# huyhoang17/DB_text_minimal

Measured on AMD Instinct MI355X. Metric: train images/sec @640x640 bs=16/GPU, higher is better.
Workload: dtype f32

## Files before the change

### db_text_minimal_amd/_lib.py

```python
import ctypes
import os
import subprocess

_HERE = os.path.dirname(os.path.abspath(__file__))
LIB_PATH = os.environ.get('DBN_LIB_PATH') or os.path.join(_HERE, 'libdbnet_hip.so')
CSRC = os.path.join(_HERE, 'csrc')

_P, _I, _L, _F, _D = ctypes.c_void_p, ctypes.c_int, ctypes.c_long, ctypes.c_float, ctypes.c_double

SIGNATURES = {
    'dbn_pack_weights': 'piiiiiipp',
    'dbn_igemm_panel_floats': 'iiiiii',
    'dbn_igemm_packed_floats': 'ii',
    'dbn_igemm_f32': 'pppp' + 'i' * 14 + 'p',
    'dbn_igemm_tile_config': 'ii',
    'dbn_igemm_tile_config_ns': 'iii',
    'dbn_conv_bn_ws_floats': 'iiiiii',
    'dbn_pack_weights_batched': 'piip',
    'dbn_igemm_splitk_plan': 'iiii',
    'dbn_igemm_splitk_plan_ns': 'iiiii',
    'dbn_igemm_splitk_f32': 'pppp' + 'i' * 16 + 'pp',
    'dbn_deform_im2col': 'ppp' + 'i' * 11 + 'p',
    'dbn_deform_col2im': 'ppppp' + 'i' + 'p' + 'i' * 11 + 'p',
    'dbn_deform_col2im_ws_bytes': 'i' * 8,
# ... 85 lines not shown
    'dbn_head_tail_bwd': 'p' * 21 + 'iiii' + 'ff' + 'pp',
    'dbn_db_loss_ws_bytes': '',
    'dbn_db_loss_fwd': 'pp' + 'iiii' + 'ffdf' + 'pppp',
    'dbn_db_loss_sum_fwd': 'pp' + 'iiii' + 'ffdf' + 'pppp',
    'dbn_db_loss_frac_fwd': 'pp' + 'iiii' + 'ffdf' + 'i' + 'pppp',
    'dbn_db_loss_bwd': 'pppp' + 'ff' + 'iiii' + 'pp',
    'dbn_db_loss_ohem_ws_bytes': 'iii',
    'dbn_db_loss_ohem_fwd': 'pp' + 'iiii' + 'ffdf' + 'pppp',
    'dbn_db_loss_ohem_bwd': 'ppppp' + 'ff' + 'iiii' + 'pp',
    'dbn_pixel_confusion': 'plppiiifpp',
    'dbn_adam_step': 'pppp' + 'l' + 'ffff' + 'i' + 'f' + 'p',
    'dbn_clock_probe': 'pip',
    'dbn_has_experiments': '',
    'dbn_wall_clock_khz': '',
}
SIGNATURES.update({
    'dbn_igemm_t': 'ii' + 'pppp' + 'i' * 14 + 'i' + 'p' + 'p',
    'dbn_conv_bn_t': 'i' + SIGNATURES['dbn_conv_bn_f32'],
    'dbn_pyramid_conv_t': 'i' + SIGNATURES['dbn_pyramid_conv_f32'],
    'dbn_pyramid_conv_from_t': 'ii' + SIGNATURES['dbn_pyramid_conv_f32'],
    'dbn_igemm_bn_rows': 'i' * 15,
    'dbn_igemm_bnsums_t': 'ii' + 'pppp' + 'i' * 14 + 'ppppppp' + 'pppp' + 'p' + 'p',
    'dbn_igemm_bn_final_counters': 'ii',
    'dbn_igemm_bn_final_group_floats': 'ii',
    'dbn_wgrad_t': 'ii' + 'pppp' + 'i' * 12 + 'f' + 'p',
    'dbn_wgrad_phase_t': 'iii' + 'pppp' + 'i' * 12 + 'f' + 'p',
    'dbn_wgrad_reduce_describe': 'ii' + 'pppp' + 'i' * 12 + 'f' + 'p',
    'dbn_wgrad_reduce_many': 'ppiiip',
    'dbn_wgrad_tile_config': 'ii',
    'dbn_set_wgrad_variant': 'i',
    'dbn_set_convt_kernel': 'i',
    'dbn_igemm_splitk_slab_floats': 'iiiii',
    'dbn_wgrad_kernel_config': 'iiiii',
    'dbn_wgrad_kernel_config_hw': 'i' * 12,
    'dbn_set_patch_conv': 'i',
    'dbn_set_wres16': 'i',
    'dbn_set_pyramid_wide': 'i',
    'dbn_pyramid_wide_would_run': 'iiiiii',
    'dbn_conv_bn_set_final': 'pp',
    'dbn_conv_bn_final_group_doubles': 'ii',
    'dbn_wres16_would_run': 'iiiiiiiii',
    'dbn_mfma_sustained': 'ippip',
    'dbn_mfma_sustained_flops': 'ii',
    'dbn_set_stagger': 'i',
    'dbn_winograd_eligible': 'iiiii',
    'dbn_winograd_panel_floats': 'ii',
    'dbn_winograd_pack': 'piiiipp',
    'dbn_winograd_rows': 'iii',
    'dbn_winograd_pack_batched': 'pip',
    'dbn_winograd_dgrad_bnsums_f32': 'ppp' + 'iiiiii' + 'pppp' + 'ppp' + 'pppp' + 'p' + 'p',
    'dbn_winograd_ws_floats': 'iiii',
    'dbn_winograd_wgrad_eligible': 'iiiiii',
    'dbn_winograd_wgrad_linear': 'ii',
    'dbn_winograd_wgrad_slab_floats': 'iiiii',
    'dbn_winograd_wgrad_f32': 'ipppppp' + 'iiiiii' + 'fp',
    'dbn_winograd_conv_bn_act_f32': 'pppppp' + 'iiiii' + 'pp' + 'ff' + 'ppppppp' + 'p',
    'dbn_winograd_conv_bn_f32': 'pppp' + 'iiiii' + 'pp' + 'ff' + 'ppppppp' + 'p',
    'dbn_set_phase_priority': 'i',
    'dbn_set_winograd_persistent': 'i',
    'dbn_set_winograd_stagger': 'i',
    'dbn_set_winograd_blocks_per_barrier': 'i',
    'dbn_fold_bn_eval': 'pilppppp' + 'f' + 'ppp',
    'dbn_igemm_act_t': 'ii' + 'pppp' + 'i' + 'p' + 'i' * 13 + 'p',
    'dbn_winograd_conv_act_f32': 'pppp' + 'i' + 'p' + 'iiiii' + 'p',
    'dbn_pyramid_conv_act_t': 'ii' + 'p' * 9 + 'i' + 'p' + 'i' * 6 + 'p',
    'dbn_set_trace': 'pl',
    'dbn_igemm_kernel_config': 'i' * 16,
    'dbn_split3': 'pplp',
    'dbn_deform_im2col_t': 'i' + SIGNATURES['dbn_deform_im2col'],
    'dbn_deform_col2im_t': 'i' + SIGNATURES['dbn_deform_col2im'],
    'dbn_deform_col2im_gather_t': 'i' + SIGNATURES['dbn_deform_col2im'],
    'dbn_deform_col2im_gather_ws_bytes': 'iii',
    'dbn_deform_offset_absmax_t': 'iplpp',
    'dbn_pw16_eligible': 'iiiiii',
    'dbn_pw16_panel_bytes': '',
    'dbn_pw16_pack': 'ipipp',
    'dbn_pw16_act_t': 'ipppipiiiip',
    'dbn_set_head_tail_wide': 'i',
    'dbn_stem16_pool_eligible': 'iiii',
    'dbn_stem16_conv_bn_relu_pool_t': 'ipppppiiip',
    'dbn_head16_eligible': 'iiii',
    'dbn_head16_tail_eval_t': 'i' + 'p' * 15 + 'iii' + 'p',
    'dbn_cast_f32': 'ipplp',
    'dbn_pack_weights_t': 'ip' + 'i' * 7 + 'pp',
    'dbn_igemm_panel_floats_t': 'i' * 8,
    'dbn_bn_train_stats_t': 'i' + SIGNATURES['dbn_bn_train_stats'],
    'dbn_bn_apply_t': 'i' + SIGNATURES['dbn_bn_apply'],
    'dbn_bn_backward_t': 'ipi' + SIGNATURES['dbn_bn_backward_ex'][1:],
    'dbn_col_sum_t': 'i' + SIGNATURES['dbn_col_sum'],
    'dbn_bnrelu_maxpool_fwd_t': 'i' + SIGNATURES['dbn_bnrelu_maxpool_fwd'],
    'dbn_bnrelu_maxpool_bwd_t': 'i' + SIGNATURES['dbn_bnrelu_maxpool_bwd'][:-1] + 'pppp',
    'dbn_maxpool_bwd_parts': 'iiii',
    'dbn_bnrelu_maxpool_fwd_arg_t': 'ipppppp' + 'iiii' + 'p',
    'dbn_maxpool_bn_backward_ws_floats': 'iiii',
    'dbn_maxpool_bn_backward_t': 'i' + 'p' * 10 + 'iiii' + 'f' + 'pp',
    'dbn_nearest_up_fwd_t': 'i' + SIGNATURES['dbn_nearest_up_fwd'],
    'dbn_nearest_up_bwd_t': 'i' + SIGNATURES['dbn_nearest_up_bwd'],
    'dbn_nchw3_to_nhwc4_t': 'i' + SIGNATURES['dbn_nchw3_to_nhwc4'],
    'dbn_nchw3_to_nhwc4_packed_t': 'i' + SIGNATURES['dbn_nchw3_to_nhwc4'],
    'dbn_nchw3_to_nhwc16_and_4_t': 'ipppiiip',
    'dbn_convt16_rows': '',
    'dbn_convt16_panel_bytes': '',
    'dbn_convt16_eligible': 'iiiiii',
    'dbn_convt16_pack': 'ippp',
    'dbn_convt16_bn_t': 'ippppiii' + 'pp' + 'ff' + 'ppppppp' + 'p',
    'dbn_stem16_padded_h': 'i',
# ... 86 lines not shown
```

### db_text_minimal_amd/csrc/winograd_wgrad_f32.hip

```cpp
#include "igemm_common.h"
#include <algorithm>
#ifndef DBN_WWG_PIPE
#define DBN_WWG_PIPE 1
#endif
#ifndef DBN_WWG_EXP
#define DBN_WWG_EXP 0
#endif

namespace {

constexpr int WG_XPX = 180, WG_XROW = 18, WG_YPX = 128, WG_YROW = 16;

struct WinoWgradParams {
    const float* x;
    const float* dy;
    float* slab;
    int N, H, W, Cx, Cy;
    int nob, nib;
    int tw, gpi, groups;
    int nsplit;
    unsigned x_bytes, dy_bytes;
    const float *x_scale, *x_shift;
};

constexpr int WL_XPX = 336, WL_YPX = 240;
template <bool LIN>
__global__ __launch_bounds__(512) __attribute__((amdgpu_waves_per_eu(2, 2))) void winograd_wgrad_f32_kernel(const WinoWgradParams p) {
    constexpr int XPX = LIN ? WL_XPX : WG_XPX, YPX = LIN ? WL_YPX : WG_YPX;
    constexpr int XCH = XPX * 16, YCH = YPX * 16;
    constexpr int NXP = (XCH + 511) / 512, NYP = (YCH + 511) / 512;
    constexpr int NBUF = LIN ? 1 : 2;
    __shared__ f32x4 smem[NBUF * (XCH + YCH)];
    const int tid = threadIdx.x, lane = tid & 63, wave = __builtin_amdgcn_readfirstlane(tid >> 6);
    const int li = lane & 31, lh = lane >> 5;
    const int irow = wave & 3, oh = wave >> 2;
    const int nsub = p.nob * p.nib;
    const int b = dbn_xcd_remap(blockIdx.x, gridDim.x);
    const int split = b / nsub, sub = b - split * nsub;
    const int ob = sub / p.nib, ib = sub - ob * p.nib;
    const int g0 = (int)((long)split * p.groups / p.nsplit), g1 = (int)((long)(split + 1) * p.groups / p.nsplit);
    const __amdgpu_buffer_rsrc_t rsX = __builtin_amdgcn_make_buffer_rsrc(const_cast<float*>(p.x), 0, p.x_bytes, 0x00020000);
    const __amdgpu_buffer_rsrc_t rsY = __builtin_amdgcn_make_buffer_rsrc(const_cast<float*>(p.dy), 0, p.dy_bytes, 0x00020000);
    const int TW = (p.W + 1) >> 1, TI = ((p.H + 1) >> 1) * TW;
    const int prow = LIN ? 2 * TW + 2 : WG_XROW, yrow = LIN ? 2 * TW : WG_YROW;
    const float rTW = 1.0f / (float)TW;

    unsigned xrel[NXP], yrel[NYP];
    int xpos[NXP], ypos[NYP];
#pragma unroll
    for (int j = 0; j < NXP; ++j) {
        const int idx = tid + j * 512, pix = idx >> 4, ch = idx & 15;
        int py, px;
        if constexpr (LIN) divmod24(pix, prow, 1.0f / (float)prow, py, px);
        else { py = pix / WG_XROW; px = pix - py * WG_XROW; }
        xrel[j] = (unsigned)((py * p.W + px) * p.Cx + ch * 4) * 4u;
        xpos[j] = idx < XCH ? (py | (px << 8)) : -1;
    }
#pragma unroll
    for (int j = 0; j < NYP; ++j) {
        const int idx = tid + j * 512, pix = idx >> 4, ch = idx & 15;
        int py, px;
        if constexpr (LIN) divmod24(pix, yrow, 1.0f / (float)yrow, py, px);
        else { py = pix >> 4; px = pix & 15; }
        yrel[j] = (unsigned)((py * p.W + px) * p.Cy + ch * 4) * 4u;
        ypos[j] = idx < YCH ? (py | (px << 8)) : -1;
    }
    f32x4 rx[NXP], ry[LIN ? 1 : NYP];
    const bool act = p.x_scale != nullptr;
    f32x4 asc_ = {0.f, 0.f, 0.f, 0.f}, ash_ = {0.f, 0.f, 0.f, 0.f};
    if (act && !LIN) {
        asc_ = *reinterpret_cast<const f32x4*>(p.x_scale + ib * 64 + (tid & 15) * 4);
        ash_ = *reinterpret_cast<const f32x4*>(p.x_shift + ib * 64 + (tid & 15) * 4);
    }
    unsigned xstatic = 0;
#pragma unroll
    for (int j = 0; j < NXP; ++j) xstatic |= (unsigned)(xpos[j] >= 0) << j;
    unsigned xvalid = 0;
    int t0 = 0, tr0 = 0;
    auto geometry = [&](int g, int& n, int& hs0, int& ws0, int& xrows) {
        n = g / p.gpi;
        const int t = g - n * p.gpi;
        if constexpr (LIN) {
            const int tfirst = t * 32, tlast = min(tfirst + 31, TI - 1);
            const int r0_ = tfirst / TW, r1_ = tlast / TW;
            hs0 = 2 * r0_ - 1;
            ws0 = -1;
            xrows = 2 * (r1_ - r0_ + 1) + 2;
        } else {
            const int ty = t / p.tw, tx = t - ty * p.tw;
            hs0 = ty * 8 - 1;
            ws0 = tx * 16 - 1;
            xrows = 10;
        }
    };
    auto load_x = [&](int g) {
        int n, hs0, ws0, xrows;
        geometry(g, n, hs0, ws0, xrows);
        const unsigned bx = (unsigned)(((n * p.H + hs0) * p.W + ws0) * p.Cx + ib * 64) * 4u;
        if (!LIN && hs0 >= 0 && hs0 + 10 <= p.H && ws0 >= 0 && ws0 + WG_XROW <= p.W) {
#pragma unroll
            for (int j = 0; j < NXP; ++j) rx[j] = buffer_load_f32x4(rsX, xpos[j] >= 0 ? bx + xrel[j] : OOB_OFFSET);
            xvalid = xstatic;
            return;
        }
#pragma unroll
        for (int j = 0; j < NXP; ++j) {
            const int py = xpos[j] & 255, px = xpos[j] >> 8;
            const bool v = xpos[j] >= 0 && py < xrows && (unsigned)(hs0 + py) < (unsigned)p.H && (unsigned)(ws0 + px) < (unsigned)p.W;
            rx[j] = buffer_load_f32x4(rsX, v ? bx + xrel[j] : OOB_OFFSET);
            xvalid = (xvalid & ~(1u << j)) | ((unsigned)v << j);
        }
    };
    int sbuf = 0;
    auto store_x = [&](int xrows) {
        f32x4* const dstX = smem + sbuf * (XCH + YCH);
        if (act) {
            const f32x4 asc = LIN ? *reinterpret_cast<const f32x4*>(p.x_scale + ib * 64 + (tid & 15) * 4) : asc_;
            const f32x4 ash = LIN ? *reinterpret_cast<const f32x4*>(p.x_shift + ib * 64 + (tid & 15) * 4) : ash_;
#pragma unroll
            for (int j = 0; j < NXP; ++j)
#pragma unroll
                for (int e = 0; e < 4; ++e) rx[j][e] = ((xvalid >> j) & 1u) ? dbn_affine_relu(rx[j][e], asc[e], ash[e]) : 0.f;
        }
#pragma unroll
        for (int j = 0; j < NXP; ++j)
            if (xpos[j] >= 0 && (xpos[j] & 255) < xrows) dstX[tid + j * 512] = rx[j];
    };
    auto y_piece = [&](int j, int n, int hs0, int ws0, int xrows) {
        const int py = ypos[j] & 255, px = ypos[j] >> 8;
        const unsigned by = (unsigned)(((n * p.H + hs0 + 1) * p.W + ws0 + 1) * p.Cy + ob * 64) * 4u;
        if (!LIN && hs0 + 9 <= p.H && ws0 + 17 <= p.W) return buffer_load_f32x4(rsY, by + yrel[j]);
        const bool v = ypos[j] >= 0 && py < xrows - 2 && hs0 + 1 + py < p.H && ws0 + 1 + px < p.W;
        return buffer_load_f32x4(rsY, v ? by + yrel[j] : OOB_OFFSET);
    };
    auto load_group = [&](int g) {
        int n, hs0, ws0, xrows;
        geometry(g, n, hs0, ws0, xrows);
        load_x(g);
        if constexpr (!LIN) {
#pragma unroll
            for (int j = 0; j < NYP; ++j) ry[j] = y_piece(j, n, hs0, ws0, xrows);
        }
    };
    auto store_group = [&]() {
        store_x(10);
        if constexpr (!LIN) {
#pragma unroll
            for (int j = 0; j < NYP; ++j) smem[sbuf * (XCH + YCH) + XCH + tid + j * 512] = ry[j];
        }
        sbuf ^= 1;
    };
    auto stage_lin = [&](int g) {
        int n, hs0, ws0, xrows;
        geometry(g, n, hs0, ws0, xrows);
        load_x(g);
        f32x4 q[4];
#pragma unroll
        for (int h = 0; h < NYP; h += 4) {
#pragma unroll
            for (int j = 0; j < 4; ++j)
                if (h + j < NYP) q[j] = y_piece(h + j, n, hs0, ws0, xrows);
            if (h == 0) store_x(xrows);
#pragma unroll
            for (int j = 0; j < 4; ++j)
                if (h + j < NYP && ypos[h + j] >= 0 && (ypos[h + j] & 255) < xrows - 2) smem[XCH + tid + (h + j) * 512] = q[j];
        }
        t0 = (g - n * p.gpi) * 32;
        tr0 = t0 / TW;
    };

    const int a1 = irow == 0 ? 0 : (irow == 2 ? 2 : 1), a2 = irow == 0 ? 2 : (irow == 1 ? 2 : (irow == 2 ? 1 : 3));
    const float sa = irow == 1 ? 1.f : -1.f;
    const float c0 = irow == 3 ? 0.f : 1.f, c1 = irow == 0 ? 0.f : (irow == 1 ? 1.f : -1.f);
    typedef float f32x2 __attribute__((ext_vector_type(2)));
    const f32x2* const X2 = reinterpret_cast<const f32x2*>(smem) + (LIN ? 0 : (2 * lh) * 32) + li;
    const f32x2* const Xr1 = X2 + a1 * prow * 32;
    const f32x2* const Xr2 = X2 + a2 * prow * 32;
    const float* const Yb = reinterpret_cast<const float*>(smem + XCH) + (LIN ? 0 : (2 * lh) * 64) + oh * 32 + li;

    f32x16 acc[4][2];
#pragma unroll
    for (int j = 0; j < 4; ++j)
#pragma unroll
        for (int h = 0; h < 2; ++h)
#pragma unroll
            for (int r = 0; r < 16; ++r) acc[j][h][r] = 0.f;

    if constexpr (!LIN) {
        if (g0 < g1) {
            load_group(g0);
            store_group();
            if (g0 + 1 < g1) load_group(g0 + 1);
        }
        __syncthreads();
    }
    for (int g = g0; g < g1; ++g) {
        int cbuf = 0;
        if constexpr (LIN) {
            if (g > g0) __syncthreads();
            stage_lin(g);
            __syncthreads();
        } else {
            cbuf = (g - g0) & 1;
            if (DBN_WWG_EXP != 1) {
                if (g + 1 < g1) store_group();
                if (g + 2 < g1) load_group(g + 2);
            }
        }
        const int xoff2 = cbuf * (XCH + YCH) * 2, yoff4 = cbuf * (XCH + YCH) * 4;
#if DBN_WWG_PIPE
        if constexpr (!LIN) {
            f32x2 U1[4], U2[4], V[4];
            float dd[4], D[4];
            auto fetch = [&](int s_) {
                const int xo = xoff2 + (2 * (s_ >> 2) * WG_XROW + 4 * (s_ & 3)) * 32, yo = yoff4 + (2 * (s_ >> 2) * WG_YROW + 4 * (s_ & 3)) * 64;
#pragma unroll
                for (int q = 0; q < 4; ++q) {
                    U1[q] = Xr1[xo + q * 32];
                    U2[q] = Xr2[xo + q * 32];
                }
                dd[0] = Yb[yo];
                dd[1] = Yb[yo + 64];
                dd[2] = Yb[yo + WG_YROW * 64];
                dd[3] = Yb[yo + WG_YROW * 64 + 64];
            };
            auto form = [&]() {
                f32x2 R[4];
#pragma unroll
                for (int q = 0; q < 4; ++q) {
                    R[q][0] = fmaf(sa, U2[q][0], U1[q][0]);
                    R[q][1] = fmaf(sa, U2[q][1], U1[q][1]);
                }
                V[0] = R[0] - R[2];
                V[1] = R[1] + R[2];
                V[2] = R[2] - R[1];
                V[3] = R[1] - R[3];
                const float r0 = fmaf(c1, dd[2], c0 * dd[0]), r1 = fmaf(c1, dd[3], c0 * dd[1]);
                D[0] = r0;
                D[1] = r0 + r1;
                D[2] = r0 - r1;
                D[3] = -r1;
            };
            fetch(0);
            form();
#pragma unroll
            for (int s = 0; s < 16; ++s) {
                f32x2 Vc[4];
                float Dc[4];
#pragma unroll
                for (int j = 0; j < 4; ++j) {
                    Vc[j] = V[j];
                    Dc[j] = D[j];
                }
                __builtin_amdgcn_sched_barrier(0);
                if (s + 1 < 16) fetch(s + 1);
                __builtin_amdgcn_sched_barrier(0);
#pragma unroll
                for (int j = 0; j < 4; ++j)
#pragma unroll
                    for (int h = 0; h < 2; ++h) acc[j][h] = __builtin_amdgcn_mfma_f32_32x32x2f32(Dc[j], Vc[j][h], acc[j][h], 0, 0, 0);
                __builtin_amdgcn_sched_barrier(0);
                if (s + 1 < 16) form();
// ... 3 lines not shown
#pragma unroll
        for (int s = 0; s < 16; ++s) {
            int xo, yo;
            float c0s = c0, c1s = c1;
            if constexpr (LIN) {
                const int t = t0 + 2 * s + lh;
                const bool ok = t < TI;
                int ty, tx;
                divmod24(ok ? t : t0, TW, rTW, ty, tx);
                ty -= tr0;
                xo = (2 * ty * prow + 2 * tx) * 32;
                yo = (2 * ty * yrow + 2 * tx) * 64;
                c0s = ok ? c0 : 0.f;
                c1s = ok ? c1 : 0.f;
            } else {
                xo = (2 * (s >> 2) * WG_XROW + 4 * (s & 3)) * 32;
                yo = (2 * (s >> 2) * WG_YROW + 4 * (s & 3)) * 64;
            }
            f32x2 R[4];
#if DBN_WWG_EXP == 2 || DBN_WWG_EXP == 6
            for (int q = 0; q < 4; ++q) { R[q][0] = rx[q][0]; R[q][1] = rx[q][1]; }
            const float d00 = rx[0][0], d01 = rx[0][1], d10 = rx[1][0], d11 = rx[1][1];
#if DBN_WWG_EXP == 6
            for (int q = 0; q < 4; ++q) { R[q][0] = fmaf(sa, rx[q][1], R[q][0]); R[q][1] = fmaf(sa, rx[q][2], R[q][1]); }
#endif
#else
#pragma unroll
            for (int q = 0; q < 4; ++q) {
                const f32x2 u1 = Xr1[xoff2 + xo + q * 32], u2 = Xr2[xoff2 + xo + q * 32];
#if DBN_WWG_EXP == 5
                R[q][0] = u1[0];
                R[q][1] = u2[1];
#else
                R[q][0] = fmaf(sa, u2[0], u1[0]);
                R[q][1] = fmaf(sa, u2[1], u1[1]);
#endif
            }
            const float* const Yc = Yb + yoff4;
            const float d00 = Yc[yo], d01 = Yc[yo + 64], d10 = Yc[yo + yrow * 64], d11 = Yc[yo + yrow * 64 + 64];
#endif
#if DBN_WWG_EXP == 2 || DBN_WWG_EXP == 5
            const f32x2 V[4] = {R[0], R[1], R[2], R[3]};
            const float D[4] = {d00, d01, d10, d11};
#else
            const f32x2 V[4] = {R[0] - R[2], R[1] + R[2], R[2] - R[1], R[1] - R[3]};
            const float r0 = fmaf(c1s, d10, c0s * d00), r1 = fmaf(c1s, d11, c0s * d01);
            const float D[4] = {r0, r0 + r1, r0 - r1, -r1};
#endif
#pragma unroll
            for (int j = 0; j < 4; ++j)
#pragma unroll
                for (int h = 0; h < 2; ++h) acc[j][h] = __builtin_amdgcn_mfma_f32_32x32x2f32(D[j], V[j][h], acc[j][h], 0, 0, 0);
        }
        if constexpr (!LIN) {
            if (g + 1 < g1 && DBN_WWG_EXP != 1) __syncthreads();
        }
    }
    float* const S = p.slab + ((long)b * 16 + 4 * irow) * 4096 + (oh * 32 + 4 * lh) * 64 + 2 * li;
#pragma unroll
    for (int j = 0; j < 4; ++j)
#pragma unroll
        for (int r = 0; r < 16; ++r) {
            f32x2 v;
            v[0] = acc[j][0][r];
            v[1] = acc[j][1][r];
            *reinterpret_cast<f32x2*>(S + j * 4096 + ((r & 3) + 8 * (r >> 2)) * 64) = v;
        }
}

__global__ __launch_bounds__(1024) void winograd_wgrad_reduce_serial_kernel(const float* __restrict__ slab, int nsplit, int nsub, int nib, int I,
                                                                     float* __restrict__ grad, float scale) {
    __shared__ double sh[16][64];
    __shared__ float st[576];
    const int o = blockIdx.x, ib = blockIdx.y, sub = (o >> 6) * nib + ib;
    const int pnt = threadIdx.x >> 6, il = threadIdx.x & 63;
    const float* src = slab + ((long)sub * 16 + pnt) * 4096 + (o & 63) * 64 + il;
    const long stride = (long)nsub * 16 * 4096;
    double s = 0.0;
    int z = 0;
    for (; z + 3 < nsplit; z += 4)
        s += ((double)src[z * stride] + (double)src[(z + 1) * stride]) + ((double)src[(z + 2) * stride] + (double)src[(z + 3) * stride]);
    for (; z < nsplit; ++z) s += (double)src[z * stride];
    sh[pnt][il] = s;
    __syncthreads();
    if (threadIdx.x < 576) {
        const int c = threadIdx.x / 9, tap = threadIdx.x - c * 9, r = tap / 3, q = tap - r * 3;
        auto gcol = [](int k, double v0, double v1, double v2, double v3) {
            return k == 0 ? v0 + 0.5 * (v1 + v2) : (k == 1 ? 0.5 * (v1 - v2) : 0.5 * (v1 + v2) + v3);
        };
        double t[4];
#pragma unroll
        for (int i = 0; i < 4; ++i) t[i] = gcol(q, sh[4 * i + 0][c], sh[4 * i + 1][c], sh[4 * i + 2][c], sh[4 * i + 3][c]);
        st[threadIdx.x] = (float)(gcol(r, t[0], t[1], t[2], t[3]) * (double)scale);
    }
    __syncthreads();
    const int n = min(64, I - ib * 64) * 9;
    float* dst = grad + ((long)o * I + ib * 64) * 9;
    for (int k = threadIdx.x; k < n; k += 1024) dst[k] = st[k];
}

template <int ZL>
__global__ __launch_bounds__(256) void winograd_wgrad_reduce_kernel(const float* __restrict__ slab, int nsplit, int nsub, int nib, int I,
                                                                    float* __restrict__ grad, float scale) {
    constexpr int OG = 32 / ZL, ZH = ZL / 2;
    __shared__ double part[ZH * OG][16][32 + 1];
    __shared__ double sh[OG][16][32];
    __shared__ float st[OG * 288];
    const int ib = blockIdx.y >> 1, ih = blockIdx.y & 1;
// ... 18 lines not shown
    }
    if (zl2 >= ZH) {
#pragma unroll
        for (int pt = 0; pt < 16; ++pt)
#pragma unroll
            for (int e = 0; e < 4; ++e) part[zl * OG + og][pt][iq * 4 + e] = acc[pt][e];
    }
    __syncthreads();
    if (zl2 < ZH) {
#pragma unroll
        for (int pt = 0; pt < 16; ++pt)
#pragma unroll
            for (int e = 0; e < 4; ++e) part[zl * OG + og][pt][iq * 4 + e] += acc[pt][e];
    }
    __syncthreads();
    for (int k = threadIdx.x; k < OG * 16 * 32; k += 256) {
        const int g = k >> 9, pt = (k >> 5) & 15, c = k & 31;
        double s_ = 0.0;
#pragma unroll
        for (int q = 0; q < ZH; ++q) s_ += part[q * OG + g][pt][c];
        sh[g][pt][c] = s_;
    }
    __syncthreads();
    for (int k = threadIdx.x; k < OG * 288; k += 256) {
        const int g = k / 288, kk = k - g * 288, c = kk / 9, tap = kk - c * 9, r = tap / 3, q = tap - r * 3;
        auto gcol = [](int w, double v0, double v1, double v2, double v3) {
            return w == 0 ? v0 + 0.5 * (v1 + v2) : (w == 1 ? 0.5 * (v1 - v2) : 0.5 * (v1 + v2) + v3);
        };
        double t[4];
#pragma unroll
        for (int i = 0; i < 4; ++i) t[i] = gcol(q, sh[g][4 * i + 0][c], sh[g][4 * i + 1][c], sh[g][4 * i + 2][c], sh[g][4 * i + 3][c]);
        st[k] = (float)(gcol(r, t[0], t[1], t[2], t[3]) * (double)scale);
    }
    __syncthreads();
    const int c0 = ib * 64 + ih * 32;
    const int n = max(0, min(32, I - c0)) * 9;
    for (int k = threadIdx.x; k < OG * n; k += 256) {
        const int g = k / n, kk = k - g * n;
        grad[((long)(blockIdx.x * OG + g) * I + c0) * 9 + kk] = st[g * 288 + kk];
    }
}

int wwg_splits(int groups, int nsub) {
    static const int wgs = dbn_env_int("DBN_WWG_WGS", 256);
    int ns = std::max(1, wgs / nsub);
    return std::min(ns, groups);
}

bool wwg_linear_fits(int H, int W) {
    const int TW = (W + 1) / 2, TH = (H + 1) / 2;
    const int R = std::min(TH, (30 + TW) / TW + 1);
    return (2 * R + 2) * (2 * TW + 2) <= WL_XPX && 2 * R * 2 * TW <= WL_YPX;
}
double wwg_fill(int H, int W, bool lin) {
    if (lin) {
        const long TI = (long)((H + 1) / 2) * ((W + 1) / 2);
        return (double)TI / (double)((TI + 31) / 32 * 32);
    }
    return (double)H * W / ((double)((H + 7) / 8 * 8) * ((W + 15) / 16 * 16));
}
bool wwg_linear(int H, int W) {
    static const int env = dbn_env_int("DBN_WWG_LIN", 1);
    return env && wwg_linear_fits(H, W) && wwg_fill(H, W, true) > wwg_fill(H, W, false) + 0.2;
}
int wwg_groups(int N, int H, int W) {
    if (wwg_linear(H, W)) return N * (int)(((long)((H + 1) / 2) * ((W + 1) / 2) + 31) / 32);
    return N * ((H + 7) / 8) * ((W + 15) / 16);
}

}

extern "C" {

int dbn_winograd_wgrad_eligible(int N, int H, int W, int O, int Cb, int I) {
    if (N < 1 || H < 1 || W < 1 || O % 64 || Cb % 64 || I < 1 || I > Cb) return 0;
    const long px = (long)N * H * W;
    if (px * std::max(O, Cb) * 4 >= dbn_g_byte_limit) return 0;
    return wwg_fill(H, W, wwg_linear(H, W)) >= 0.5;
}
int dbn_winograd_wgrad_linear(int H, int W) { return wwg_linear(H, W); }
long dbn_winograd_wgrad_slab_floats(int N, int H, int W, int O, int Cb) {
    const int nsub = (O / 64) * (Cb / 64);
    return (long)wwg_splits(wwg_groups(N, H, W), nsub) * nsub * 16 * 4096;
}
int dbn_winograd_wgrad_f32(int phases, const float* dy, const float* x, const float* x_scale, const float* x_shift, float* slab, float* grad,
                           int N, int H, int W, int O, int Cb, int I, float scale, void* stream) {
    DBN_REQUIRE(dy && x && slab && grad && phases >= 1 && phases <= 3 && !x_scale == !x_shift);
    DBN_REQUIRE(dbn_winograd_wgrad_eligible(N, H, W, O, Cb, I));
    WinoWgradParams p;
    p.x = x;
    p.dy = dy;
    p.slab = slab;
    p.x_scale = x_scale;
    p.x_shift = x_shift;
    p.N = N;
    p.H = H;
    p.W = W;
    p.Cx = Cb;
    p.Cy = O;
    p.nob = O / 64;
    p.nib = Cb / 64;
    const bool lin = wwg_linear(H, W);
    p.tw = (W + 15) / 16;
    p.groups = wwg_groups(N, H, W);
    p.gpi = p.groups / N;
    p.nsplit = wwg_splits(p.groups, p.nob * p.nib);
    p.x_bytes = (unsigned)((long)N * H * W * Cb * 4);
    p.dy_bytes = (unsigned)((long)N * H * W * O * 4);
    hipStream_t st = (hipStream_t)stream;
    if (phases & 1) {
        const dim3 grid(p.nsplit * p.nob * p.nib);
        if (lin) hipLaunchKernelGGL(winograd_wgrad_f32_kernel<true>, grid, dim3(512), 0, st, p);
        else hipLaunchKernelGGL(winograd_wgrad_f32_kernel<false>, grid, dim3(512), 0, st, p);
    }
    if (phases & 2) {
        const int nsub = p.nob * p.nib;
        if (p.nsplit >= 128)
            hipLaunchKernelGGL(winograd_wgrad_reduce_kernel<32>, dim3(O, 2 * p.nib), dim3(256), 0, st, slab, p.nsplit, nsub, p.nib, I, grad, scale);
        else
            hipLaunchKernelGGL(winograd_wgrad_reduce_serial_kernel, dim3(O, p.nib), dim3(1024), 0, st, slab, p.nsplit, nsub, p.nib, I, grad, scale);
    }
    return dbn_status();
}

}
```

### db_text_minimal_amd/engine.py

```python
import contextlib
import ctypes
import os

import torch

from . import _lib
from ._lib import check

DEAD_PREFIXES = ('backbone.fc.', 'backbone.smooth.')
K_STEP_DEFAULT = 50.0


def _p(t):
    return None if t is None else t.data_ptr()


def _out_hw(conv, H, W):
    k, s, p = conv.k, conv.stride, conv.padding
    return (H + 2 * p - k) // s + 1, (W + 2 * p - k) // s + 1


NO_BN = (None, None, 0.0, 0.0) + (None, ) * 7


# ... 48 lines not shown
        e1 = torch.cuda.Event(enable_timing=True)
        e0.record()
        self._open = (label, flops, nbytes, e0, e1, tag)

    def end(self):
        if self._open is not None:
            self._open[4].record()
            self.records.append(self._open)
            self._open = None

    def summary(self, peak_tflops=None, hbm_gbs=None):
        out = {}
        for label, flops, nbytes, e0, e1, _ in self.records:
            d = out.setdefault(label, dict(launches=0, ms=0.0, flops=0.0, bytes=0.0, roof_ms=0.0, hbm_bound=0))
            d['launches'] += 1
            d['ms'] += e0.elapsed_time(e1)
            d['flops'] += flops
            d['bytes'] += nbytes
            if peak_tflops and hbm_gbs and flops > 0:
                t_m, t_h = flops / (peak_tflops * 1e9), nbytes / (hbm_gbs * 1e6)
                d['roof_ms'] += max(t_m, t_h)
                d['hbm_bound'] += int(t_h > t_m)
        return out


class _VirtualConv:

    def __init__(self, cin, cout, k, stride, padding, weight, bias):
        self.cin, self.cout, self.k, self.stride, self.padding, self.weight, self.bias = cin, cout, k, stride, padding, weight, bias


class ConvPlan(object):
    __slots__ = ('winograd', 'winograd_wgrad', 'apply_on_load', 'fold', 'pw16')


class _Shape:

    def __init__(self, *shape):
        self.shape = shape


class Engine:
    def __init__(self, model):
        self.model = model
        self.L = _lib.lib()
        if 'DBN_PATCH_F32' in os.environ:
            self.L.dbn_set_patch_conv(2 if os.environ['DBN_PATCH_F32'] == '0' else 3)
        if 'DBN_WINO_PERSISTENT' in os.environ:
            self.L.dbn_set_winograd_persistent(int(os.environ['DBN_WINO_PERSISTENT']))
        if 'DBN_WINO_CBS' in os.environ:
            self.L.dbn_set_winograd_blocks_per_barrier(int(os.environ['DBN_WINO_CBS']))
        if 'DBN_WINO_STAGGER' in os.environ:
            self.L.dbn_set_winograd_stagger(int(os.environ['DBN_WINO_STAGGER']))
        if 'DBN_PHASE_PRIO' in os.environ:
            self.L.dbn_set_phase_priority(int(os.environ['DBN_PHASE_PRIO']))
        if 'DBN_STAGGER' in os.environ:
            self.L.dbn_set_stagger(int(os.environ['DBN_STAGGER']))
        self.bufs = {}
        self.packs = {}
        self.pack_src = {}
        self._pack_jobs = None
        self.param_epoch = 0
        self.generation = 0
        self.saved_generation = -1
        self.flat = None
        self.flat_grad = None
        self.offsets = None
        self.views = {}
        self.grad_views = {}
        self._dcn_slots, self._dcn_E = {}, {}
        self._plans = {}
        self.dcn_forms = {'gather': 0, 'scatter': 0}
        self.grad_scale = 1.0
        self._live = None
        self.nbt_pending = {}
        self._bias_done = set()
        self._bnb_sums = {}
        self._reduce_pending = []
        self._wgrad_fifo = []
        self._wino_src = {}
        self._wino_jobs = None
        self._reduce_job_cache = {}
        self._reduce_tables = {}
        self._by_ptr = {}
        self._plane_cache = {}
        self.presplit = os.environ.get('DBN_PRESPLIT', '0') == '1' and bool(self.L.dbn_has_experiments())
        self.prof = None
        self.grad_ready_hook = None
        self.ns = 0
        self.at = 0
        self.overlap_wgrad = True
        self.overlap_head_branches = os.environ.get('DBN_OVERLAP_HEAD', '0') == '1'
        self.side_priority = None
        self._side = None
        self._side_used = False
        self._slab_free = [None, None]

    @property
    def live_params(self):
        if self._live is None:
            self._live = [(n, p) for n, p in self.model.named_parameters() if not n.startswith(DEAD_PREFIXES)]
        return self._live

    def ensure_flat(self):
        params = self.live_params
        dev = params[0][1].device
# ... 1757 lines not shown
```

### include/dbnet_hip.h

```cpp
#ifndef DBNET_HIP_H
#define DBNET_HIP_H
#ifdef __cplusplus
extern "C" {
#endif


int dbn_pack_weights(const float* w_oihw, int O, int I, int R, int S, int mode, int stride, float* out, void* stream);
long dbn_igemm_panel_floats(int O, int I, int R, int S, int mode, int stride);
int dbn_igemm_packed_floats(int K, int Cd);

int dbn_igemm_f32(const float* src, const float* wpk, const float* bias, float* dst, int N, int Hs, int Ws, int Cs, int Hd,
                  int Wd, int Cd, int R, int S, int stride, int pad, int mode, int accumulate, int tile_hint, void* stream);

int dbn_pack_weights_bf16s(const float* w_oihw, int O, int I, int R, int S, int mode, int stride, int ns, float* out, void* stream);
int dbn_pack_weights_batched(const void* jobs, int n, int ns, void* stream);
long dbn_igemm_bf16s_panel_floats(int O, int I, int R, int S, int mode, int stride, int ns);
int dbn_igemm_bf16s(const float* src, const float* wpk, const float* bias, float* dst, int N, int Hs, int Ws, int Cs, int Hd,
                    int Wd, int Cd, int R, int S, int stride, int pad, int mode, int accumulate, int tile_hint, int ns,
                    void* stream);
int dbn_wgrad_bf16s(const float* sm, const float* big, float* slab, float* grad_oihw, int N, int Ho, int Wo, int O, int H, int W,
                    int Cb, int I, int R, int S, int stride, int pad, float scale, int ns, void* stream);

int dbn_igemm_bn_rows(int at, int ns, int N, int Hs, int Ws, int Cs, int Hd, int Wd, int Cd, int R, int S, int stride, int pad, int mode,
                      int tile_hint);
// ... 79 lines not shown
int dbn_bnrelu_maxpool_fwd(const float* y, const float* scale, const float* shift, float* out, int N, int H, int W, int C,
                           void* stream);
int dbn_bnrelu_maxpool_bwd(const float* y, const float* scale, const float* shift, const float* pooled, const float* dpool,
                           float* dz, int N, int H, int W, int C, void* stream);

int dbn_nearest_up_fwd(const float* src, const float* addend, float* dst, int N, int Hs, int Ws, int C, int H, int W, int Cdst,
                       int coff, void* stream);
int dbn_nearest_up_bwd(const float* dbig, float* dsrc, int N, int Hs, int Ws, int C, int H, int W, int Cbig, int coff,
                       int accumulate, void* stream);

int dbn_bilinear_fwd(const float* src, float* dst, long planes, int Hs, int Ws, int H, int W, void* stream);
int dbn_bilinear_bwd(const float* ddst, float* dsrc, long planes, int Hs, int Ws, int H, int W, void* stream);

int dbn_fpn_combine_weights(const float* w, int Co, int Cin, int group, int Cg, float* wd, void* stream);
int dbn_fpn_scatter_wgrad(const float* t0, const float* t1, const float* t2, const float* t3, int Co, int Cg, float* dw,
                          void* stream);

int dbn_nchw3_to_nhwc4(const float* x, float* out, int N, int H, int W, void* stream);
int dbn_add_inplace(const float* x, float* y, long n, void* stream);

int dbn_head_tail_fwd(const float* xb, const float* xt, const float* wb, const float* wt, const float* bias_b,
                      const float* bias_t, const float* bn_scale_b, const float* bn_shift_b, const float* bn_scale_t,
                      const float* bn_shift_t, float* out, int N, int Hq, int Wq, int channels, float kstep, void* stream);
int dbn_head_tail_bwd_ws_floats(void);
int dbn_head_tail_bwd(const float* xb, const float* xt, const float* wb, const float* wt, const float* preds,
                      const float* dpreds, const float* bn_scale_b, const float* bn_shift_b, const float* bn_scale_t,
                      const float* bn_shift_t, const float* bn_mean_b, const float* bn_rstd_b, const float* bn_mean_t,
                      const float* bn_rstd_t, float* bn_sums, float* dxb, float* dxt, float* dw_b, float* dbias_b, float* dw_t,
                      float* dbias_t, int N, int Hq, int Wq, int channels, float kstep, float grad_scale, float* ws, void* stream);

int dbn_set_winograd_persistent(int on);
int dbn_set_winograd_stagger(int permille);
int dbn_set_winograd_blocks_per_barrier(int n);
int dbn_winograd_eligible(int N, int H, int W, int Cs, int Cd);
long dbn_winograd_panel_floats(int O, int Cs);
int dbn_winograd_pack(const float* w_oihw, int O, int I, int Cs, int dgrad, float* out, void* stream);
int dbn_winograd_pack_batched(const void* jobs, int n, void* stream);
int dbn_winograd_rows(int N, int H, int W);
int dbn_winograd_dgrad_bnsums_f32(const float* dy, const float* upanel, float* dx, int N, int H, int W, int Cs, int Cd, int accumulate,
                                  const void* y, const void* zmask, const float* mask_scale, const float* mask_shift,
                                  const float* save_mean, const float* save_rstd, float* part, const void* y2, const float* save_mean2,
                                  const float* save_rstd2, float* part2, const dbn_bnb_final* fin, void* stream);
long dbn_winograd_ws_floats(int N, int H, int W, int Cd);
int dbn_winograd_conv_bn_act_f32(const float* src, const float* in_scale, const float* in_shift, const float* upanel, const float* bias,
                                 float* dst, int N, int H, int W, int Cs, int Cd, const float* gamma, const float* beta, float eps,
                                 float momentum, float* run_mean, float* run_var, float* scale, float* shift, float* save_mean,
                                 float* save_rstd, float* ws, void* stream);
int dbn_winograd_conv_bn_f32(const float* src, const float* upanel, const float* bias, float* dst, int N, int H, int W, int Cs, int Cd,
                             const float* gamma, const float* beta, float eps, float momentum, float* run_mean, float* run_var,
                             float* scale, float* shift, float* save_mean, float* save_rstd, float* ws, void* stream);

int dbn_winograd_wgrad_eligible(int N, int H, int W, int O, int Cb, int I);
int dbn_winograd_wgrad_linear(int H, int W);
long dbn_winograd_wgrad_slab_floats(int N, int H, int W, int O, int Cb);
int dbn_winograd_wgrad_f32(int phases, const float* dy, const float* x, const float* x_scale, const float* x_shift, float* slab, float* grad,
                           int N, int H, int W, int O, int Cb, int I, float scale, void* stream);

int dbn_db_loss_ws_bytes(void);
int dbn_db_loss_fwd(const float* preds, const float* gts, int N, int H, int W, int channels, float alpha, float beta,
                    double negative_ratio, float eps, float* losses, float* coef, void* ws, void* stream);
int dbn_db_loss_bwd(const float* preds, const float* gts, const float* coef, const float* grad_losses, float alpha, float beta,
                    int N, int H, int W, int channels, float* dpreds, void* stream);
int dbn_db_loss_sum_fwd(const float* preds, const float* gts, int N, int H, int W, int channels, float alpha, float beta,
                        double negative_ratio, float eps, float* losses, float* coef, void* ws, void* stream);
int dbn_db_loss_frac_fwd(const float* preds, const float* gts, int N, int H, int W, int channels, float alpha, float beta,
                         double negative_ratio, float eps, int sum, float* losses, float* coef, void* ws, void* stream);

long dbn_db_loss_ohem_ws_bytes(int N, int H, int W);
int dbn_db_loss_ohem_fwd(const float* preds, const float* gts, int N, int H, int W, int channels, float alpha, float beta,
                         double negative_ratio, float eps, float* losses, float* coef, void* ws, void* stream);
int dbn_db_loss_ohem_bwd(const float* preds, const float* gts, const float* coef, const float* grad_losses, const void* ws,
                         float alpha, float beta, int N, int H, int W, int channels, float* dpreds, void* stream);

int dbn_pixel_confusion(const float* preds, long batch_stride, const float* gt, const float* mask, int N, int H, int W, float thresh,
                        double* hist, void* stream);

int dbn_adam_step(float* p, const float* g, float* m, float* v, long n, float lr, float beta1, float beta2, float eps, int step,
                  float grad_scale, void* stream);

int dbn_has_experiments(void);

int dbn_clock_probe(void* out2, int microseconds, void* stream);
int dbn_wall_clock_khz(void);

int dbn_deform_im2col(const float* x, const float* offset, float* cols, int N, int H, int W, int C, int Ho, int Wo, int R, int S,
                      int stride, int pad, int off_stride, void* stream);
long dbn_deform_col2im_ws_bytes(int N, int H, int W, int C, int Ho, int Wo, int R, int S);
int dbn_deform_col2im(const float* dcols, const float* x, const float* offset, float* dx, float* doffset, int accumulate, void* ws, int N,
                      int H, int W, int C, int Ho, int Wo, int R, int S, int stride, int pad, int off_stride, void* stream);
int dbn_permute_weight(const float* src, float* dst, int O, int C, int T, int to_ohwi, float scale, void* stream);

int dbn_binarize_u8(const float* pred, int N, int channels, int H, int W, float thresh, unsigned char* out, void* stream);
int dbn_box_scores(const float* bitmap, int H, int W, const float* boxes, int K, int P, float* scores, void* stream);

int dbn_gt_maps(const double* verts, const double* dist, const int* meta, const int* img_off, const int* ixy, int N, int P, int S,
                int max_verts, int max_off_pts, float scale, float tmin, float* out, void* stream);
int dbn_normalize_u8(const unsigned char* in, int N, int H, int W, float m0, float m1, float m2, float* out, void* stream);
int dbn_poly_offset(const double* xy, int n, const double* delta, int* out_xy, int cap, int* out_n);
int dbn_poly_offset_paths(const double* xy, int n, const double* delta, int* out_xy, int cap, int* out_n, int* out_paths);

int dbn_warp_affine_u8(const unsigned char* src, long src_bytes, const long long* desc, const double* coef, int N, int max_h, int max_w,
                       unsigned char* dst, long dst_bytes, void* stream);
int dbn_resize_cubic_u8(const unsigned char* src, long src_bytes, const long long* desc, const double* coef, int N, int max_h, int max_w,
                        unsigned char* dst, long dst_bytes, void* stream);
int dbn_resize_linear_norm_u8(const unsigned char* src, long src_bytes, const long long* desc, const double* coef, int N, int CH, int CW,
                              float m0, float m1, float m2, float* out, void* stream);
// ... 238 lines not shown
```

Baseline: 745.3.

## Add double-buffered pipelined schedule for linear-layout Winograd wgrad kernel

Adds a pipelined variant of the linear (small-spatial) Winograd weight-gradient kernel. Each 32-tile group is split into two 16-tile halves with smaller shared-memory footprints, so the next half can be prefetched into a second buffer while MFMAs run on the current one. This replaces the old single-buffer stage/sync/compute sequence. An even-tile-width specialization lets both lane halves walk the same tiles. It is enabled by default when the geometry fits, at the cost of more barriers per group and extra complexity in the validity masks.

```diff
diff --git a/db_text_minimal_amd/_lib.py b/db_text_minimal_amd/_lib.py
--- a/db_text_minimal_amd/_lib.py
+++ b/db_text_minimal_amd/_lib.py
@@ -161,6 +161,8 @@
     'dbn_winograd_ws_floats': 'iiii',
     'dbn_winograd_wgrad_eligible': 'iiiiii',
     'dbn_winograd_wgrad_linear': 'ii',
+    'dbn_set_wwg_lin_pipe': 'i',
+    'dbn_winograd_wgrad_lin_pipelined': 'ii',
     'dbn_winograd_wgrad_slab_floats': 'iiiii',
     'dbn_winograd_wgrad_f32': 'ipppppp' + 'iiiiii' + 'fp',
     'dbn_winograd_conv_bn_act_f32': 'pppppp' + 'iiiii' + 'pp' + 'ff' + 'ppppppp' + 'p',
diff --git a/db_text_minimal_amd/csrc/winograd_wgrad_f32.hip b/db_text_minimal_amd/csrc/winograd_wgrad_f32.hip
--- a/db_text_minimal_amd/csrc/winograd_wgrad_f32.hip
+++ b/db_text_minimal_amd/csrc/winograd_wgrad_f32.hip
@@ -24,12 +24,16 @@
 };
 
 constexpr int WL_XPX = 336, WL_YPX = 240;
-template <bool LIN>
+constexpr int WP_XPX = 176, WP_YPX = 120;
+template <bool LIN, int LPM = 0>
 __global__ __launch_bounds__(512) __attribute__((amdgpu_waves_per_eu(2, 2))) void winograd_wgrad_f32_kernel(const WinoWgradParams p) {
-    constexpr int XPX = LIN ? WL_XPX : WG_XPX, YPX = LIN ? WL_YPX : WG_YPX;
+    constexpr bool LP = LPM != 0, EV = LPM == 2;
+    static_assert(LIN || !LP, "LP is a schedule of the LIN form");
+    constexpr bool PRE = !LIN || LP;
+    constexpr int XPX = LP ? WP_XPX : (LIN ? WL_XPX : WG_XPX), YPX = LP ? WP_YPX : (LIN ? WL_YPX : WG_YPX);
     constexpr int XCH = XPX * 16, YCH = YPX * 16;
     constexpr int NXP = (XCH + 511) / 512, NYP = (YCH + 511) / 512;
-    constexpr int NBUF = LIN ? 1 : 2;
+    constexpr int NBUF = PRE ? 2 : 1;
     __shared__ f32x4 smem[NBUF * (XCH + YCH)];
     const int tid = threadIdx.x, lane = tid & 63, wave = __builtin_amdgcn_readfirstlane(tid >> 6);
     const int li = lane & 31, lh = lane >> 5;
@@ -65,10 +69,16 @@
         yrel[j] = (unsigned)((py * p.W + px) * p.Cy + ch * 4) * 4u;
         ypos[j] = idx < YCH ? (py | (px << 8)) : -1;
     }
-    f32x4 rx[NXP], ry[LIN ? 1 : NYP];
+    const int pix0 = tid >> 4;
+    unsigned xcol = 0, ycol = 0;
+#pragma unroll
+    for (int j = 0; j < NXP; ++j) xcol |= (unsigned)(xpos[j] >= 0 && (unsigned)((xpos[j] >> 8) - 1) < (unsigned)p.W) << j;
+#pragma unroll
+    for (int j = 0; j < NYP; ++j) ycol |= (unsigned)(ypos[j] >= 0 && (ypos[j] >> 8) < p.W) << j;
+    f32x4 rx[NXP], ry[PRE ? NYP : 1];
     const bool act = p.x_scale != nullptr;
     f32x4 asc_ = {0.f, 0.f, 0.f, 0.f}, ash_ = {0.f, 0.f, 0.f, 0.f};
-    if (act && !LIN) {
+    if (act && PRE) {
         asc_ = *reinterpret_cast<const f32x4*>(p.x_scale + ib * 64 + (tid & 15) * 4);
         ash_ = *reinterpret_cast<const f32x4*>(p.x_shift + ib * 64 + (tid & 15) * 4);
     }
@@ -78,14 +88,15 @@
     unsigned xvalid = 0;
     int t0 = 0, tr0 = 0;
     auto geometry = [&](int g, int& n, int& hs0, int& ws0, int& xrows) {
-        n = g / p.gpi;
-        const int t = g - n * p.gpi;
+        const int gg = LP ? g >> 1 : g;
+        n = gg / p.gpi;
+        const int t = gg - n * p.gpi;
         if constexpr (LIN) {
-            const int tfirst = t * 32, tlast = min(tfirst + 31, TI - 1);
+            const int tfirst = LP ? t * 32 + (g & 1) * 16 : t * 32, tlast = min(tfirst + (LP ? 15 : 31), TI - 1);
             const int r0_ = tfirst / TW, r1_ = tlast / TW;
             hs0 = 2 * r0_ - 1;
             ws0 = -1;
-            xrows = 2 * (r1_ - r0_ + 1) + 2;
+            xrows = !LP || tfirst < TI ? 2 * (r1_ - r0_ + 1) + 2 : 0;
         } else {
             const int ty = t / p.tw, tx = t - ty * p.tw;
             hs0 = ty * 8 - 1;
@@ -103,6 +114,17 @@
             xvalid = xstatic;
             return;
         }
+        if constexpr (LP) {
+            const int lo = hs0 < 0 ? prow : 0, hi = min(xrows, p.H - hs0) * prow;
+#pragma unroll
+            for (int j = 0; j < NXP; ++j) {
+                const int pix = pix0 + 32 * j;
+                const bool v = ((xcol >> j) & 1u) && pix >= lo && pix < hi;
+                rx[j] = buffer_load_f32x4(rsX, v ? bx + xrel[j] : OOB_OFFSET);
+                xvalid = (xvalid & ~(1u << j)) | ((unsigned)v << j);
+            }
+            return;
+        }
 #pragma unroll
         for (int j = 0; j < NXP; ++j) {
             const int py = xpos[j] & 255, px = xpos[j] >> 8;
@@ -115,8 +137,8 @@
     auto store_x = [&](int xrows) {
         f32x4* const dstX = smem + sbuf * (XCH + YCH);
         if (act) {
-            const f32x4 asc = LIN ? *reinterpret_cast<const f32x4*>(p.x_scale + ib * 64 + (tid & 15) * 4) : asc_;
-            const f32x4 ash = LIN ? *reinterpret_cast<const f32x4*>(p.x_shift + ib * 64 + (tid & 15) * 4) : ash_;
+            const f32x4 asc = !PRE ? *reinterpret_cast<const f32x4*>(p.x_scale + ib * 64 + (tid & 15) * 4) : asc_;
+            const f32x4 ash = !PRE ? *reinterpret_cast<const f32x4*>(p.x_shift + ib * 64 + (tid & 15) * 4) : ash_;
 #pragma unroll
             for (int j = 0; j < NXP; ++j)
 #pragma unroll
@@ -124,31 +146,47 @@
         }
 #pragma unroll
         for (int j = 0; j < NXP; ++j)
-            if (xpos[j] >= 0 && (xpos[j] & 255) < xrows) dstX[tid + j * 512] = rx[j];
+            if (LP ? tid + j * 512 < XCH : xpos[j] >= 0 && (xpos[j] & 255) < xrows) dstX[tid + j * 512] = rx[j];
     };
     auto y_piece = [&](int j, int n, int hs0, int ws0, int xrows) {
-        const int py = ypos[j] & 255, px = ypos[j] >> 8;
         const unsigned by = (unsigned)(((n * p.H + hs0 + 1) * p.W + ws0 + 1) * p.Cy + ob * 64) * 4u;
         if (!LIN && hs0 + 9 <= p.H && ws0 + 17 <= p.W) return buffer_load_f32x4(rsY, by + yrel[j]);
+        if constexpr (LP) {
+            const bool v = ((ycol >> j) & 1u) && pix0 + 32 * j < min(xrows - 2, p.H - hs0 - 1) * yrow;
+            return buffer_load_f32x4(rsY, v ? by + yrel[j] : OOB_OFFSET);
+        }
+        const int py = ypos[j] & 255, px = ypos[j] >> 8;
         const bool v = ypos[j] >= 0 && py < xrows - 2 && hs0 + 1 + py < p.H && ws0 + 1 + px < p.W;
         return buffer_load_f32x4(rsY, v ? by + yrel[j] : OOB_OFFSET);
     };
+    int rrows = 10;
     auto load_group = [&](int g) {
         int n, hs0, ws0, xrows;
         geometry(g, n, hs0, ws0, xrows);
         load_x(g);
-        if constexpr (!LIN) {
+        if constexpr (PRE) {
 #pragma unroll
             for (int j = 0; j < NYP; ++j) ry[j] = y_piece(j, n, hs0, ws0, xrows);
         }
+        if constexpr (LP) rrows = xrows;
     };
     auto store_group = [&]() {
+        if constexpr (LP) {
+            if (rrows == 0) return false;
+            store_x(rrows);
+#pragma unroll
+            for (int j = 0; j < NYP; ++j)
+                if (tid + j * 512 < YCH) smem[sbuf * (XCH + YCH) + XCH + tid + j * 512] = ry[j];
+            sbuf ^= 1;
+            return true;
+        }
         store_x(10);
         if constexpr (!LIN) {
 #pragma unroll
             for (int j = 0; j < NYP; ++j) smem[sbuf * (XCH + YCH) + XCH + tid + j * 512] = ry[j];
         }
         sbuf ^= 1;
+        return true;
     };
     auto stage_lin = [&](int g) {
         int n, hs0, ws0, xrows;
@@ -173,10 +211,10 @@
     const float sa = irow == 1 ? 1.f : -1.f;
     const float c0 = irow == 3 ? 0.f : 1.f, c1 = irow == 0 ? 0.f : (irow == 1 ? 1.f : -1.f);
     typedef float f32x2 __attribute__((ext_vector_type(2)));
-    const f32x2* const X2 = reinterpret_cast<const f32x2*>(smem) + (LIN ? 0 : (2 * lh) * 32) + li;
+    const f32x2* const X2 = reinterpret_cast<const f32x2*>(smem) + (LIN && !EV ? 0 : (2 * lh) * 32) + li;
     const f32x2* const Xr1 = X2 + a1 * prow * 32;
     const f32x2* const Xr2 = X2 + a2 * prow * 32;
-    const float* const Yb = reinterpret_cast<const float*>(smem + XCH) + (LIN ? 0 : (2 * lh) * 64) + oh * 32 + li;
+    const float* const Yb = reinterpret_cast<const float*>(smem + XCH) + (LIN && !EV ? 0 : (2 * lh) * 64) + oh * 32 + li;
 
     f32x16 acc[4][2];
 #pragma unroll
@@ -186,28 +224,116 @@
 #pragma unroll
             for (int r = 0; r < 16; ++r) acc[j][h][r] = 0.f;
 
-    if constexpr (!LIN) {
-        if (g0 < g1) {
-            load_group(g0);
+    const int s0 = LP ? 2 * g0 : g0, s1 = LP ? 2 * g1 : g1;
+    if constexpr (PRE) {
+        if (s0 < s1) {
+            load_group(s0);
             store_group();
-            if (g0 + 1 < g1) load_group(g0 + 1);
+            if (s0 + 1 < s1) load_group(s0 + 1);
         }
         __syncthreads();
     }
-    for (int g = g0; g < g1; ++g) {
+    int lbuf = 0;
+    for (int g = s0; g < s1; ++g) {
         int cbuf = 0;
-        if constexpr (LIN) {
+        bool next_staged = true;
+        if constexpr (LIN && !LP) {
             if (g > g0) __syncthreads();
             stage_lin(g);
             __syncthreads();
         } else {
-            cbuf = (g - g0) & 1;
+            cbuf = LP ? lbuf : (g - g0) & 1;
             if (DBN_WWG_EXP != 1) {
-                if (g + 1 < g1) store_group();
-                if (g + 2 < g1) load_group(g + 2);
+                if (g + 1 < s1) next_staged = store_group();
+                if (g + 2 < s1) load_group(g + 2);
             }
         }
         const int xoff2 = cbuf * (XCH + YCH) * 2, yoff4 = cbuf * (XCH + YCH) * 4;
+        if constexpr (LP) {
+            const int gg = g >> 1, tg = (gg - gg / p.gpi * p.gpi) * 32 + (g & 1) * 16;
+            const int nreal = max(0, min(16, TI - tg)), tc = nreal ? tg : tg - 16;
+            const int tx0 = tc - tc / TW * TW;
+            const int xob = xoff2 + 2 * tx0 * 32, yob = yoff4 + 2 * tx0 * 64;
+            const int dxw = (2 * prow - 2 * TW + 4) * 32, dyw = (2 * yrow - 2 * TW + 4) * 64, yr64 = yrow * 64;
+            const int lhv = EV ? 0 : lh;
+            const int lim = nreal - lhv;
+            int tx = tx0 + lhv;
+            const bool w0 = tx >= TW;
+            tx -= w0 ? TW : 0;
+            int xo = xob + (w0 ? 2 * prow * 32 : 0) + 2 * (tx - tx0) * 32, yo = yob + (w0 ? 2 * yrow * 64 : 0) + 2 * (tx - tx0) * 64;
+            f32x2 U1[4], U2[4], V[4];
+            float dd[4], D[4], k0 = 0.f, k1 = 0.f;
+            auto fetch = [&](int s_) {
+                const bool ok = 2 * s_ < lim;
+                const int xs = ok ? xo : xob, ys = ok ? yo : yob;
+                k0 = ok ? c0 : 0.f;
+                k1 = ok ? c1 : 0.f;
+#pragma unroll
+                for (int q = 0; q < 4; ++q) {
+                    U1[q] = Xr1[xs + q * 32];
+                    U2[q] = Xr2[xs + q * 32];
+                }
+                dd[0] = Yb[ys];
+                dd[1] = Yb[ys + 64];
+                dd[2] = Yb[ys + yr64];
+                dd[3] = Yb[ys + yr64 + 64];
+                tx += 2;
+                const bool w = tx >= TW;
+                tx -= w ? TW : 0;
+                xo += w ? dxw : 4 * 32;
+                yo += w ? dyw : 4 * 64;
+            };
+            auto form = [&]() {
+                f32x2 R[4];
+#pragma unroll
+                for (int q = 0; q < 4; ++q) {
+                    R[q][0] = fmaf(sa, U2[q][0], U1[q][0]);
+                    R[q][1] = fmaf(sa, U2[q][1], U1[q][1]);
+                }
+                V[0] = R[0] - R[2];
+                V[1] = R[1] + R[2];
+                V[2] = R[2] - R[1];
+                V[3] = R[1] - R[3];
+                const float r0 = fmaf(k1, dd[2], k0 * dd[0]), r1 = fmaf(k1, dd[3], k0 * dd[1]);
+                D[0] = r0;
+                D[1] = r0 + r1;
+                D[2] = r0 - r1;
+                D[3] = -r1;
+            };
+#if DBN_WWG_PIPE
+            fetch(0);
+            form();
+#pragma unroll
+            for (int s = 0; s < 8; ++s) {
+                f32x2 Vc[4];
+                float Dc[4];
+#pragma unroll
+                for (int j = 0; j < 4; ++j) {
+                    Vc[j] = V[j];
+                    Dc[j] = D[j];
+                }
+                __builtin_amdgcn_sched_barrier(0);
+                if (s + 1 < 8) fetch(s + 1);
+                __builtin_amdgcn_sched_barrier(0);
+#pragma unroll
+                for (int j = 0; j < 4; ++j)
+#pragma unroll
+                    for (int h = 0; h < 2; ++h) acc[j][h] = __builtin_amdgcn_mfma_f32_32x32x2f32(Dc[j], Vc[j][h], acc[j][h], 0, 0, 0);
+                __builtin_amdgcn_sched_barrier(0);
+                if (s + 1 < 8) form();
+            }
+#else
+#pragma unroll
+            for (int s = 0; s < 8; ++s) {
+                fetch(s);
+                form();
+#pragma unroll
+                for (int j = 0; j < 4; ++j)
+#pragma unroll
+                    for (int h = 0; h < 2; ++h) acc[j][h] = __builtin_amdgcn_mfma_f32_32x32x2f32(D[j], V[j][h], acc[j][h], 0, 0, 0);
+            }
+#endif
+        } else
 #if DBN_WWG_PIPE
         if constexpr (!LIN) {
             f32x2 U1[4], U2[4], V[4];
@@ -317,8 +443,9 @@
 #pragma unroll
                 for (int h = 0; h < 2; ++h) acc[j][h] = __builtin_amdgcn_mfma_f32_32x32x2f32(D[j], V[j][h], acc[j][h], 0, 0, 0);
         }
-        if constexpr (!LIN) {
-            if (g + 1 < g1 && DBN_WWG_EXP != 1) __syncthreads();
+        if constexpr (PRE) {
+            if (g + 1 < s1 && DBN_WWG_EXP != 1) __syncthreads();
+            if constexpr (LP) lbuf ^= (int)next_staged;
         }
     }
     float* const S = p.slab + ((long)b * 16 + 4 * irow) * 4096 + (oh * 32 + 4 * lh) * 64 + 2 * li;
@@ -443,6 +570,13 @@
     const int R = std::min(TH, (30 + TW) / TW + 1);
     return (2 * R + 2) * (2 * TW + 2) <= WL_XPX && 2 * R * 2 * TW <= WL_YPX;
 }
+bool wwg_lin_pipe_fits(int H, int W) {
+    const int TW = (W + 1) / 2, TH = (H + 1) / 2;
+    const int R = std::min(TH, (14 + TW) / TW + 1);
+    return TW >= 2 && (2 * R + 2) * (2 * TW + 2) <= WP_XPX && 2 * R * 2 * TW <= WP_YPX;
+}
+int g_wwg_lin_pipe = 1;
+bool wwg_lin_pipe() { return g_wwg_lin_pipe != 0; }
 double wwg_fill(int H, int W, bool lin) {
     if (lin) {
         const long TI = (long)((H + 1) / 2) * ((W + 1) / 2);
@@ -470,6 +604,11 @@
     return wwg_fill(H, W, wwg_linear(H, W)) >= 0.5;
 }
 int dbn_winograd_wgrad_linear(int H, int W) { return wwg_linear(H, W); }
+int dbn_set_wwg_lin_pipe(int on) {
+    g_wwg_lin_pipe = on != 0;
+    return DBN_OK;
+}
+int dbn_winograd_wgrad_lin_pipelined(int H, int W) { return wwg_linear(H, W) && wwg_lin_pipe() && wwg_lin_pipe_fits(H, W); }
 long dbn_winograd_wgrad_slab_floats(int N, int H, int W, int O, int Cb) {
     const int nsub = (O / 64) * (Cb / 64);
     return (long)wwg_splits(wwg_groups(N, H, W), nsub) * nsub * 16 * 4096;
@@ -501,8 +640,11 @@
     hipStream_t st = (hipStream_t)stream;
     if (phases & 1) {
         const dim3 grid(p.nsplit * p.nob * p.nib);
-        if (lin) hipLaunchKernelGGL(winograd_wgrad_f32_kernel<true>, grid, dim3(512), 0, st, p);
-        else hipLaunchKernelGGL(winograd_wgrad_f32_kernel<false>, grid, dim3(512), 0, st, p);
+        const bool pipe = lin && wwg_lin_pipe() && wwg_lin_pipe_fits(H, W);
+        if (pipe && ((W + 1) / 2) % 2 == 0) hipLaunchKernelGGL((winograd_wgrad_f32_kernel<true, 2>), grid, dim3(512), 0, st, p);
+        else if (pipe) hipLaunchKernelGGL((winograd_wgrad_f32_kernel<true, 1>), grid, dim3(512), 0, st, p);
+        else if (lin) hipLaunchKernelGGL((winograd_wgrad_f32_kernel<true, 0>), grid, dim3(512), 0, st, p);
+        else hipLaunchKernelGGL((winograd_wgrad_f32_kernel<false, 0>), grid, dim3(512), 0, st, p);
     }
     if (phases & 2) {
         const int nsub = p.nob * p.nib;
diff --git a/db_text_minimal_amd/engine.py b/db_text_minimal_amd/engine.py
--- a/db_text_minimal_amd/engine.py
+++ b/db_text_minimal_amd/engine.py
@@ -124,6 +124,8 @@
             self.L.dbn_set_winograd_blocks_per_barrier(int(os.environ['DBN_WINO_CBS']))
         if 'DBN_WINO_STAGGER' in os.environ:
             self.L.dbn_set_winograd_stagger(int(os.environ['DBN_WINO_STAGGER']))
+        if 'DBN_WWG_LIN_PIPE' in os.environ:
+            self.L.dbn_set_wwg_lin_pipe(int(os.environ['DBN_WWG_LIN_PIPE']))
         if 'DBN_PHASE_PRIO' in os.environ:
             self.L.dbn_set_phase_priority(int(os.environ['DBN_PHASE_PRIO']))
         if 'DBN_STAGGER' in os.environ:
diff --git a/include/dbnet_hip.h b/include/dbnet_hip.h
--- a/include/dbnet_hip.h
+++ b/include/dbnet_hip.h
@@ -155,6 +155,8 @@
 
 int dbn_winograd_wgrad_eligible(int N, int H, int W, int O, int Cb, int I);
 int dbn_winograd_wgrad_linear(int H, int W);
+int dbn_set_wwg_lin_pipe(int on);
+int dbn_winograd_wgrad_lin_pipelined(int H, int W);
 long dbn_winograd_wgrad_slab_floats(int N, int H, int W, int O, int Cb);
 int dbn_winograd_wgrad_f32(int phases, const float* dy, const float* x, const float* x_scale, const float* x_shift, float* slab, float* grad,
                            int N, int H, int W, int O, int Cb, int I, float scale, void* stream);
```

After: 748.9 (median of 6 runs). Within noise of the previous version (+0.5%).
